# burritojustice/reporter

Measured on AMD Instinct MI355X. Metric: GPS points matched/sec (whole node) at 1/2/4/8 MI355X; % segment-ID agreement vs meili, higher is better.
Workload: dtype f32

## Files before the change

reporter_amd/csrc/engine.cpp:

```cpp
#include "engine.h"

#include "flush.h"

#include <algorithm>
#include <chrono>
#include <cmath>
#include <cstdlib>

#include <cstring>

namespace otm {

#define HIPCHK(x)                                                              \
  do {                                                                         \
    hipError_t e_ = (x);                                                       \
    if (e_ != hipSuccess) {                                                    \
      *err = std::string(#x) + ": " + hipGetErrorString(e_);                   \
      return OTM_EDEVICE;                                                      \
    }                                                                          \
  } while (0)

#define TRY(x)                    \
  do {                            \
    if (int rc_ = (x)) return rc_; \
// ... 87 lines not shown
  UP(OTMG_SHAPE_LON, s_lon);
  UP(OTMG_SHAPE_CUM, s_cum);
  UP(OTMG_SEG_ID, g_id);
  UP(OTMG_SEG_LEN, g_len);
  UP(OTMG_EDGE_HEAD_OUT, e_head_out);
  UP(OTMG_EDGE_HEAD_IN, e_head_in);
#undef UP
  {
    uint32_t tu[TURN_TABLE];
    for (int d = 0; d < TURN_TABLE; ++d) tu[d] = turn_units(E->mc.turn_penalty_factor, d);
    TRY(up(tu, sizeof tu, sizeof tu, E->dp.turn_units));
  }
  {
    const float* len = (const float*)E->host.section(OTMG_EDGE_LEN);
    std::vector<uint32_t> l64((size_t)h.n_edges + 1, 0u);
    for (int32_t e = 0; e < h.n_edges; ++e) l64[(size_t)e] = (uint32_t)std::floor((double)len[e] * 64.0 + 0.5);
    TRY(up(l64.data(), l64.size() * 4, l64.size() * 4, g.e_len64));
  }
  {
    const float* len = (const float*)E->host.section(OTMG_EDGE_LEN);
    const int32_t* seg = (const int32_t*)E->host.section(OTMG_EDGE_SEG);
    const int32_t* pos = (const int32_t*)E->host.section(OTMG_EDGE_SEG_POS);
    const uint8_t* fl = (const uint8_t*)E->host.section(OTMG_EDGE_FLAGS);
    const int64_t* way = (const int64_t*)E->host.section(OTMG_EDGE_WAY);
    std::vector<int64_t> ways(way, way + h.n_edges);
    std::sort(ways.begin(), ways.end());
    ways.erase(std::unique(ways.begin(), ways.end()), ways.end());
    if (ways.size() >= (size_t)INT32_MAX) {
      *err = "graph: more than 2^31 distinct way ids";
      return OTM_EINVAL;
    }
    std::vector<uint32_t> rec((size_t)h.n_edges * 4 + 4, 0u);
    for (int32_t e = 0; e < h.n_edges; ++e) {
      if (seg[e] >= 0 && (pos[e] < 0 || pos[e] >= (1 << 24))) {
        *err = "graph: an edge's position in its OSMLR segment exceeds 2^24";
        return OTM_EINVAL;
      }
      uint32_t* r = &rec[(size_t)e * 4];
      std::memcpy(&r[0], &len[e], 4);
      r[1] = (uint32_t)seg[e];
      r[2] = ((uint32_t)(seg[e] >= 0 ? pos[e] : 0) & 0xFFFFFFu) | ((uint32_t)fl[e] << 24);
      r[3] = (uint32_t)(std::lower_bound(ways.begin(), ways.end(), way[e]) - ways.begin());
    }
    if (ways.empty()) ways.push_back(0);
    TRY(up(rec.data(), rec.size() * 4, rec.size() * 4, g.e_rec));
    TRY(up(ways.data(), ways.size() * 8, ways.size() * 8, g.way_tab));
    const int32_t* from = (const int32_t*)E->host.section(OTMG_EDGE_FROM);
    std::vector<int32_t> fl2((size_t)h.n_edges * 2 + 2, 0);
    for (int32_t e = 0; e < h.n_edges; ++e) {
      fl2[(size_t)e * 2] = from[e];
      std::memcpy(&fl2[(size_t)e * 2 + 1], &len[e], 4);
    }
    TRY(up(fl2.data(), fl2.size() * 4, fl2.size() * 4, g.e_fl));
  }
  {
    const int m = E->grid_mult < 1 ? 1 : E->grid_mult;
    const int64_t* fo = (const int64_t*)E->host.section(OTMG_CELL_OFF);
    const uint32_t* fe = (const uint32_t*)E->host.section(OTMG_CELL_ENT);
    const int32_t R = (h.grid_rows + m - 1) / m, Cn = (h.grid_cols + m - 1) / m;
    std::vector<uint64_t> co_ent;
    const size_t nc = (size_t)R * (size_t)Cn + 1;
    std::vector<uint32_t> c32(nc, 0);
    std::vector<uint32_t> ent;
    if (m == 1) {
      if ((uint64_t)h.n_cell_entries >= (1ull << 32)) {
        *err = "graph: more than 2^32 cell entries (32-bit cell offsets)";
        return OTM_EINVAL;
      }
      for (size_t c = 0; c < nc; ++c) c32[c] = (uint32_t)fo[c];
      ent.assign(fe, fe + h.n_cell_entries);
    } else {
      co_ent.reserve((size_t)h.n_cell_entries);
      for (int32_t r = 0; r < h.grid_rows; ++r)
        for (int32_t c = 0; c < h.grid_cols; ++c) {
          const size_t f = (size_t)r * h.grid_cols + c;
          const uint64_t cc = (uint64_t)(r / m) * (uint64_t)Cn + (uint64_t)(c / m);
          for (int64_t q = fo[f]; q < fo[f + 1]; ++q) co_ent.push_back(cc << 32 | fe[q]);
        }
      std::sort(co_ent.begin(), co_ent.end());
      co_ent.erase(std::unique(co_ent.begin(), co_ent.end()), co_ent.end());
      if (co_ent.size() >= (1ull << 32)) {
        *err = "graph: more than 2^32 cell entries (32-bit cell offsets)";
        return OTM_EINVAL;
      }
      ent.resize(co_ent.size());
      for (size_t k = 0; k < co_ent.size(); ++k) {
        ent[k] = (uint32_t)co_ent[k];
        c32[(co_ent[k] >> 32) + 1]++;
      }
      for (size_t c = 0; c + 1 < nc; ++c) c32[c + 1] += c32[c];
      std::vector<uint64_t>().swap(co_ent);
    }
    E->grid_rows = R;
    E->grid_cols = Cn;
    E->grid_entries = (int64_t)ent.size();
    TRY(up(c32.data(), nc * 4, nc * 4, g.cell_off));
    TRY(up(ent.data(), ent.size() * 4, ent.size() * 4 + 16, g.cell_ent));
    const size_t ne = ent.size();
    const int32_t* soff = (const int32_t*)E->host.section(OTMG_EDGE_SHAPE_OFF);
    const float* slat = (const float*)E->host.section(OTMG_SHAPE_LAT);
    const float* slon = (const float*)E->host.section(OTMG_SHAPE_LON);
    std::vector<float> geo(ne * 4 + 4);
    for (size_t q = 0; q < ne; ++q) {
      const int32_t a = soff[ent[q] >> 4] + (int32_t)(ent[q] & 15u);
      geo[q * 4 + 0] = slat[a];
      geo[q * 4 + 1] = slon[a];
// ... 1766 lines not shown
```

reporter_amd/csrc/kernels.h:

```cpp
#pragma once
#include <hip/hip_runtime.h>

#include <cstddef>
#include <cstdint>

#include "otmatch.h"
#include "pairs.h"

namespace otm {

constexpr int KMAX = 32;
constexpr int KIN = 8;
static_assert(KIN == 4 || KIN == 8, "inline blocks of 4 or 8 slots (whole 16-B emission pieces)");
constexpr int KX = KMAX - KIN;
constexpr int MAX_HITS = 256;
constexpr int SEARCH_LIMIT = 98304;
constexpr int LDS_TABLE_CAP = 256;
constexpr int LDS_TABLE_LIMIT = 192;
constexpr int BIG_TABLE_LOG2 = 17;
constexpr int BIG_TABLE_CAP = 1 << BIG_TABLE_LOG2;
#ifndef OTM_BIG_SLOTS
#define OTM_BIG_SLOTS 512
#endif
constexpr int BIG_SLOTS = OTM_BIG_SLOTS;
constexpr int HUGE_SLOTS = 8;
constexpr int CAND_BIG_SLOTS = 64;
constexpr int HUGE_MAX_LOG2 = 27, CAND_MAX_LOG2 = 23;
__host__ __device__ inline int huge_limit(int log2) { return log2 > 2 ? 3 << (log2 - 2) : 0; }

struct DevGraph {
  const float *node_lat, *node_lon;
  const int32_t* out_off;
  const int32_t *e_from, *e_to;
  const float* e_len;
  const int32_t* e_shape_off;
  const int64_t* e_way;
  const int32_t *e_seg, *e_seg_pos;
  const uint8_t* e_flags;
  const float *s_lat, *s_lon, *s_cum;
  const uint64_t* g_id;
  const float* g_len;
  const uint32_t* cell_off;
  const uint32_t* cell_ent;
  const float4* ent_geo;
  const uint16_t *e_head_out, *e_head_in;
  const uint32_t* e_len64;
  const uint4* e_rec;
  const int2* e_fl;
  const int64_t* way_tab;
  int32_t n_nodes, n_edges, n_segments, grid_rows, grid_cols;
  double lat0, lon0, cell;
  float bb_lat0, bb_lon0, bb_inv_h, bb_inv_w;
};

#ifndef OTM_ORDER_BITS
#define OTM_ORDER_BITS 6
#endif
constexpr int ORDER_BITS = OTM_ORDER_BITS;
constexpr int ORDER_SIDE = 1 << ORDER_BITS;
constexpr int ORDER_TILES = ORDER_SIDE * ORDER_SIDE;
constexpr int ORDER_GROUPS = 8;
struct DevOrder {
  int32_t* item;
  int32_t* grp;
  uint16_t* tile;
  int32_t* tile_cnt;
  int32_t* cursor;
};

struct IdxRow {
  int64_t off;
  int32_t cnt;
  uint32_t cap;
};
#ifndef OTM_SRC_REC_BYTES
#define OTM_SRC_REC_BYTES 48
#endif
struct alignas(16) SrcRec {
  IdxRow edge;
  IdxRow node;
  int32_t from;
  int32_t len;
  int32_t pad[(OTM_SRC_REC_BYTES - 40) / 4];
};
static_assert(sizeof(SrcRec) == OTM_SRC_REC_BYTES && (OTM_SRC_REC_BYTES == 48 || OTM_SRC_REC_BYTES == 64),
              "source records of 48 or 64 bytes");
struct DevIndex {
  float rmax;
  uint32_t cmax;
  const IdxRow* row;
  const SrcRec* src;
  const uint4* slot;
  int load_pct;
};
constexpr int IDX_SLOT_BYTES = 16;
constexpr float INDEX_RMAX_CAP = 200000.0f;
constexpr uint32_t NODE_KEY = 0x80000000u;
constexpr uint32_t NONE_PRED = 0xFFFFFFFFu;
constexpr int NEAR_LEVELS = 3;
#ifndef OTM_INDEX_NEAR_FRACS
#define OTM_INDEX_NEAR_FRACS {0.45f}
// ... 298 lines not shown
```

reporter_amd/csrc/kernels.hip:

```cpp
#include <hip/hip_runtime.h>

#include <algorithm>
#include <cstdlib>
#include <type_traits>

#include <hipcub/hipcub.hpp>

#include "kernels.h"
#include "otmatch.h"

namespace otm {

namespace {

#define MPD_F 111319.4954833f
constexpr uint32_t EMPTY = 0xFFFFFFFFu;
constexpr unsigned long long LAB_NONE = ~0ull;
constexpr int TB = 64;
__device__ __forceinline__ void wave_sync() {
  __builtin_amdgcn_wave_barrier();
  asm volatile("" ::: "memory");
}

__device__ __forceinline__ float cos_deg(float deg) {
// ... 3 lines not shown
  c = c * x2 + 2.08767569878681e-09f;
  c = c * x2 - 2.755731922398589e-07f;
  c = c * x2 + 2.48015873015873e-05f;
  c = c * x2 - 0.001388888888888889f;
  c = c * x2 + 0.041666666666666664f;
  c = c * x2 - 0.5f;
  c = c * x2 + 1.0f;
  return c;
}

__device__ __forceinline__ float gc_dist(float la, float lo, float lb, float lob) {
  const float ls = MPD_F * cos_deg((la + lb) * 0.5f);
  const float dx = (lob - lo) * ls;
  const float dy = (lb - la) * MPD_F;
  return sqrtf(dx * dx + dy * dy);
}

__device__ __forceinline__ float seg_sqdist(float alat, float alon, float blat, float blon, float lat, float lon,
                                            float ls) {
  const float ax = (alon - lon) * ls;
  const float ay = (alat - lat) * MPD_F;
  const float bx = (blon - lon) * ls;
  const float by = (blat - lat) * MPD_F;
  const float vx = bx - ax;
  const float vy = by - ay;
  const float l2 = vx * vx + vy * vy;
  const float dot = ax * vx + ay * vy;
  float t = -dot / l2;
  t = t < 0.0f ? 0.0f : (t > 1.0f ? 1.0f : t);
  t = l2 > 0.0f ? t : 0.0f;
  const float px = ax + t * vx;
  const float py = ay + t * vy;
  return px * px + py * py;
}

typedef float float2_t __attribute__((ext_vector_type(2)));
__device__ __forceinline__ float seg_sqdist_pk(const float4 G, float2_t ll, float2_t sc) {
  const float2_t a = (float2_t{G.x, G.y} - ll) * sc;
  const float2_t b = (float2_t{G.z, G.w} - ll) * sc;
  const float2_t v = b - a;
  const float2_t vv = v * v;
  const float l2 = vv.y + vv.x;
  const float2_t av = a * v;
  const float dot = av.y + av.x;
  float t = -dot / l2;
  t = t < 0.0f ? 0.0f : (t > 1.0f ? 1.0f : t);
  t = l2 > 0.0f ? t : 0.0f;
  const float2_t p = a + t * v;
  const float2_t pp = p * p;
  return pp.y + pp.x;
}


struct ProjIn {
  float alon, alat, blon, blat, ca, cb, len;
  int32_t b, last;
};
__device__ __forceinline__ ProjIn proj_load(const DevGraph& g, int32_t e, int32_t k) {
  ProjIn in;
  const int32_t a = g.e_shape_off[e] + k, b = a + 1;
  in.last = g.e_shape_off[e + 1] - 1;
  in.alon = g.s_lon[a];
  in.alat = g.s_lat[a];
  in.blon = g.s_lon[b];
  in.blat = g.s_lat[b];
  in.ca = g.s_cum[a];
  in.cb = g.s_cum[b];
  in.len = g.e_len[e];
  in.b = b;
  return in;
}
__device__ __forceinline__ void proj_calc(const ProjIn& in, float lat, float lon, float ls, float& sqd,
                                          float& off_out, bool& at_end) {
  const float ax = (in.alon - lon) * ls;
  const float ay = (in.alat - lat) * MPD_F;
  const float bx = (in.blon - lon) * ls;
  const float by = (in.blat - lat) * MPD_F;
  const float vx = bx - ax;
  const float vy = by - ay;
  const float l2 = vx * vx + vy * vy;
  float t = 0.0f;
  if (l2 > 0.0f) {
    const float dot = ax * vx + ay * vy;
    t = -dot / l2;
    t = t < 0.0f ? 0.0f : (t > 1.0f ? 1.0f : t);
  }
  const float px = ax + t * vx;
  const float py = ay + t * vy;
  sqd = px * px + py * py;
  float off = in.ca + t * (in.cb - in.ca);
  off_out = off > in.len ? in.len : off;
  at_end = t == 1.0f && in.b == in.last;
}
__device__ __forceinline__ void project(const DevGraph& g, int32_t e, int32_t k, float lat, float lon, float ls,
                                        float& sqd, float& off_out, bool& at_end) {
  proj_calc(proj_load(g, e, k), lat, lon, ls, sqd, off_out, at_end);
}
__device__ __forceinline__ void project(const DevGraph& g, int32_t e, int32_t k, float lat, float lon, float ls,
                                        float& sqd, float& off_out) {
  bool at_end;
  project(g, e, k, lat, lon, ls, sqd, off_out, at_end);
}
__device__ __forceinline__ int32_t snap_node(const DevGraph& g, int32_t e, float off, bool at_end) {
  if (off == 0.0f) return g.e_from[e];
  if (at_end) {
    const int32_t v = g.e_to[e];
    if (g.out_off[v + 1] > g.out_off[v]) return v;
  }
  return -1;
}

__device__ __forceinline__ float probe_radius(const DevParams& P, float acc) {
  const float a = acc > 0.0f ? acc : P.gps_accuracy;
  const float r = a > P.search_radius ? a : P.search_radius;
  return r < P.max_search_radius ? r : P.max_search_radius;
}

__device__ __forceinline__ uint32_t fbits(float f) { return __float_as_uint(f); }
__device__ __forceinline__ float bitsf(uint32_t u) { return __uint_as_float(u); }
__device__ __forceinline__ uint32_t hash32(uint32_t x) { return x * 2654435761u; }

__device__ __forceinline__ void cadd(unsigned long long* c, unsigned long long v) {
  if (c && v) atomicAdd(c, v);
}

__device__ __forceinline__ int2 crec(const DevWork& w, int64_t p, int j) {
  return j < KIN ? w.cand_eo[p * KIN + j] : w.cand_xeo[p * KX + (j - KIN)];
}
__device__ __forceinline__ float cemis(const DevWork& w, int64_t p, int j) {
  return j < KIN ? w.cand_em[p * KIN + j] : w.cand_xem[p * KX + (j - KIN)];
}
__device__ __forceinline__ void cput(const DevWork& w, int64_t p, int j, int32_t e, float off, float em) {
  if (j < KIN) {
    w.cand_eo[p * KIN + j] = make_int2(e, __float_as_int(off));
    w.cand_em[p * KIN + j] = em;
  } else {
    w.cand_xeo[p * KX + (j - KIN)] = make_int2(e, __float_as_int(off));
    w.cand_xem[p * KX + (j - KIN)] = em;
  }
}

__device__ __forceinline__ uint32_t turn_deg(uint32_t hin, uint32_t hout) {
  int d = (int)hout - (int)hin;
  d += d < 0 ? 360 : 0;
  return (uint32_t)(d <= 180 ? d : 360 - d);
}
__device__ __forceinline__ float trans_cost(uint32_t units, float r, float gcv, float beta) {
  units = units > TURN_UNITS_MAX ? TURN_UNITS_MAX : units;
  const float tc = (float)units * 0.015625f;
  const float diff = fabsf(r - gcv);
  return (tc + diff) / beta;
}

constexpr uint32_t NO_HEAD = 0xFFFFu;
__device__ __forceinline__ bool cand_node(float off) { return off == 0.0f; }
__device__ __forceinline__ int32_t src_node(const DevGraph& g, int32_t e, float off) {
  return cand_node(off) ? g.e_from[e] : g.e_to[e];
}
__device__ __forceinline__ float src_start(const DevGraph& g, int32_t e, float off) {
  return cand_node(off) ? 0.0f : g.e_len[e] - off;
}
__device__ __forceinline__ uint32_t src_head(const DevGraph& g, int32_t e, float off) {
  return cand_node(off) ? NO_HEAD : (uint32_t)g.e_head_in[e];
}
// ... 375 lines not shown
      const uint32_t tot = e2 + (rg + 2 <= r1 ? qb[2] - qa[2] : 0u);
      const uint32_t b2 = qa[2] - e2, d1 = qa[1] - e1 - b2, d0 = qa[0] - (qa[1] - e1);
      if (CTR) ents += (unsigned long long)tot;
      auto entry_of = [&](uint32_t i) { return (size_t)(uint32_t)(i + b2 + (i < e2 ? d1 : 0u) + (i < e1 ? d0 : 0u)); };
      for (uint32_t done = 0, cn; done < tot && !spill; done += cn) {
        cn = tot - done < W ? tot - done : W;
        unsigned long long hit = 0ull;
        for (uint32_t k = 0; k < cn; k += CAND_INFL) {
          float4 G[CAND_INFL];
#pragma unroll
          for (int u = 0; u < CAND_INFL; ++u) G[u] = g.ent_geo[entry_of(done + k + (u == 0 || k + u < cn ? u : 0))];
          __builtin_amdgcn_sched_barrier(0);
          uint32_t bits = 0u;
#pragma unroll
          for (int u = 0; u < CAND_INFL; ++u) {
            const float sq = seg_sqdist_pk(G[u], pll, psc);
            bits |= ((uint32_t)(u == 0 || k + u < cn) & (uint32_t)(sq <= r2)) << u;
          }
          hit |= (unsigned long long)bits << k;
        }
        while (hit != 0ull && !spill) {
          const size_t qx = entry_of(done + (uint32_t)(__ffsll(hit) - 1));
          hit &= hit - 1ull;
          const bool two = hit != 0ull;
          const size_t qy = two ? entry_of(done + (uint32_t)(__ffsll(hit) - 1)) : qx;
          hit &= hit - 1ull;
          const uint32_t ent0 = g.cell_ent[qx], ent1 = g.cell_ent[qy];
          const float4 G0 = g.ent_geo[qx], G1 = g.ent_geo[qy];
          __builtin_amdgcn_sched_barrier(0);
          const float s0 = seg_sqdist_pk(G0, pll, psc), s1 = seg_sqdist_pk(G1, pll, psc);
          insert(ent0, s0);
          if (two && !spill) insert(ent1, s1);
        }
      }
    }
    if (spill) {
      spill_push<CTR_CAND_WAVE>(w, (int32_t)p);
      continue;
    }
    float offr[CAND_LANE_CAP];
    uint32_t perm = 076543210u;
#pragma unroll
    for (int m0 = 0; m0 < CAND_LANE_CAP; m0 += SNAP_B) {
#pragma unroll
      for (int u = 0; u < SNAP_B; ++u) offr[m0 + u] = 0.0f;
      if (m0 >= n) continue;
      uint32_t em[SNAP_B];
      ProjIn pin[SNAP_B];
#pragma unroll
      for (int u = 0; u < SNAP_B; ++u) {
        em[u] = m0 + u < n ? E[(m0 + u) * S] : 0u;
        if (m0 + u < n) pin[u] = proj_load(g, (int32_t)(em[u] >> 4), (int32_t)(em[u] & 15u));
      }
      int32_t vx[SNAP_B];
      bool node0[SNAP_B], at_end[SNAP_B];
      float offv[SNAP_B];
#pragma unroll
      for (int u = 0; u < SNAP_B; ++u) {
        vx[u] = 0;
        node0[u] = at_end[u] = false;
        offv[u] = 0.0f;
        if (m0 + u < n) {
          float sqd, off;
          proj_calc(pin[u], lat, lon, ls, sqd, off, at_end[u]);
          offv[u] = off;
          node0[u] = off == 0.0f;
          const int32_t e = (int32_t)(em[u] >> 4);
          if (node0[u] || at_end[u]) vx[u] = node0[u] ? g.e_from[e] : g.e_to[e];
        }
      }
#pragma unroll
      for (int u = 0; u < SNAP_B; ++u) {
        if (node0[u] || at_end[u]) {
          const int32_t o0 = g.out_off[vx[u]], o1 = g.out_off[vx[u] + 1];
          if (node0[u] || o1 > o0) {
            E[(m0 + u) * S] = NODE_ENT | ((uint32_t)o0 << 4);
            offv[u] = 0.0f;
          }
        }
        offr[m0 + u] = offv[u];
      }
    }
    for (int m = 0; m < n; ++m) {
      const uint32_t key = E[m * S];
      if (!(key & NODE_ENT)) continue;
      int f = -1;
      for (int t = 0; t < m; ++t)
        if (E[t * S] == key) f = t;
      if (f >= 0) {
        const float qm = Q[m * S];
        if (qm < Q[f * S]) Q[f * S] = qm;
        --n;
        E[m * S] = E[n * S];
        Q[m * S] = Q[n * S];
        perm = (perm & ~(7u << (3 * m))) | ((perm >> (3 * n)) & 7u) << (3 * m);
        --m;
      }
    }
    const int K = n < P.max_candidates ? n : P.max_candidates;
    const float ds = (2.0f * P.sigma_z) * P.sigma_z;
    for (int j = 0; j < K; ++j) {
      int m = j;
      float qm = Q[j * S];
      uint32_t em = E[j * S];
      for (int t = j + 1; t < n; ++t) {
        const float qt = Q[t * S];
        const uint32_t et = E[t * S];
        const uint32_t xt = (et & ~NODE_ENT) >> 4, xm = (em & ~NODE_ENT) >> 4;
        if (qt < qm || (qt == qm && (xt < xm || (xt == xm && et > em)))) {
          m = t;
          qm = qt;
          em = et;
        }
      }
      if (m != j) {
        Q[m * S] = Q[j * S];
        E[m * S] = E[j * S];
        Q[j * S] = qm;
        E[j * S] = em;
        const uint32_t x = ((perm >> (3 * m)) ^ (perm >> (3 * j))) & 7u;
        perm ^= x << (3 * m) | x << (3 * j);
      }
    }
    int4* eo4 = (int4*)(w.cand_eo + p * KIN);
    float4* em4 = (float4*)(w.cand_em + p * KIN);
    float emv[4];
#pragma unroll
    for (int j = 0; j < (CAND_LANE_CAP > KIN ? CAND_LANE_CAP : KIN); j += 2) {
      if (j >= KIN && j >= K) break;
      int32_t e2[2];
      float o2[2];
#pragma unroll
      for (int u = 0; u < 2; ++u) {
// ... 103 lines not shown
    const float r = probe_radius(P, pr.z);
    const float r2 = r * r;
    const float ls = MPD_F * cos_deg(lat);
    const float dlat = r / MPD_F;
    const float dlon = r / ls;
    const double la_lo = ((double)lat - (double)dlat - g.lat0) / g.cell;
    const double la_hi = ((double)lat + (double)dlat - g.lat0) / g.cell;
    const double lo_lo = ((double)lon - (double)dlon - g.lon0) / g.cell;
    const double lo_hi = ((double)lon + (double)dlon - g.lon0) / g.cell;
    const double R = g.grid_rows, Cn = g.grid_cols;
    int r0 = 0, r1 = -1, c0 = 0, c1 = -1;
    if (!(la_hi < 0.0 || lo_hi < 0.0 || la_lo >= R || lo_lo >= Cn)) {
      r0 = la_lo < 0.0 ? 0 : (int)floor(la_lo);
      r1 = la_hi >= R ? (int)R - 1 : (int)floor(la_hi);
      c0 = lo_lo < 0.0 ? 0 : (int)floor(lo_lo);
      c1 = lo_hi >= Cn ? (int)Cn - 1 : (int)floor(lo_hi);
    }
    const int ncols = c1 - c0 + 1;
    const int ncells = (r1 - r0 + 1) * ncols;
    for (int i = lane; i < hcap; i += TB) {
      Mem<BIG>::st(&hkey[i], (uint32_t)EMPTY);
      Mem<BIG>::st(&hval[i], (unsigned long long)LAB_NONE);
    }
    if (lane == 0) {
      s_count = 0;
      s_over = 0;
      s_n = 0;
    }
    __syncthreads();
    unsigned long long scanned = 0;
    for (int cb = 0; cb < ncells; cb += TB) {
      const int c = cb + lane;
      int cnt = 0;
      int64_t cs = 0;
      if (c < ncells) {
        const int rr = r0 + c / ncols, cc = c0 + c % ncols;
        const size_t cidx = (size_t)rr * (size_t)g.grid_cols + (size_t)cc;
        cs = g.cell_off[cidx];
        cnt = (int)(g.cell_off[cidx + 1] - cs);
      }
      const int incl = wave_incl_scan(cnt, lane);
      const int total = __shfl(incl, 63, 64);
      cexcl[lane] = incl - cnt;
      cstart[lane] = cs;
      __syncthreads();
      const int nc_here = min(TB, ncells - cb);
      for (int gi = lane; gi < total; gi += TB) {
        int lo = 0, hi = nc_here - 1;
        while (lo < hi) {
          const int mid = (lo + hi + 1) >> 1;
          if (cexcl[mid] <= gi) lo = mid;
          else hi = mid - 1;
        }
        const uint32_t ent = g.cell_ent[cstart[lo] + (gi - cexcl[lo])];
        const int32_t e = (int32_t)(ent >> 4), k = (int32_t)(ent & 15u);
        float sqd, off;
        project(g, e, k, lat, lon, ls, sqd, off);
        if (!(sqd <= r2)) continue;
        uint32_t slot = hash32((uint32_t)e) >> (32 - hlog2);
        bool placed = false;
        for (int probe = 0; probe < hcap; ++probe) {
          const uint32_t old = atomicCAS(&hkey[slot], EMPTY, (uint32_t)e);
          if (old == EMPTY) {
            if (atomicAdd(&s_count, 1) >= max_hits) s_over = 1;
            placed = true;
            break;
          }
          if (old == (uint32_t)e) {
            placed = true;
            break;
          }
          slot = (slot + 1) & (uint32_t)(hcap - 1);
        }
        if (!placed) {
          s_over = 1;
          continue;
        }
        atomicMin(&hval[slot], ((unsigned long long)fbits(sqd) << 32) | (unsigned long long)k);
      }
      scanned += (unsigned long long)total;
      __syncthreads();
    }
    if (s_over) {
      if (lane == 0) {
        if (!BIG) {
          spill_push<CTR_CAND_BIG>(w, (int32_t)p);
        } else if (w.cand_final) {
          w.ncand[p] = 0;
          atomicCAS(&w.trace_err[w.pt_trace[p]], 0, OTM_TERR_CAND_OVERFLOW);
        } else {
          w.ncand[p] = 0;
          w.counters_i32[CTR_GROW_CAND] = 1;
          *w.abort = 1;
        }
      }
      __syncthreads();
      continue;
    }
    for (int i = lane; i < hcap; i += TB) {
      const uint32_t hk = Mem<BIG>::ld(&hkey[i]);
      if (hk != EMPTY) {
        const unsigned long long hv = Mem<BIG>::ld(&hval[i]);
        const int idx = atomicAdd(&s_n, 1);
        Mem<BIG>::st(&skey[idx],
                     (hv & 0xFFFFFFFF00000000ull) | ((unsigned long long)hk << 5) | ((hv & 15ull) << 1));
      }
    }
    __syncthreads();
    for (int i = lane; i < hcap; i += TB) {
      Mem<BIG>::st(&hkey[i], (uint32_t)EMPTY);
      Mem<BIG>::st(&hval[i], (unsigned long long)LAB_NONE);
    }
    if (lane == 0) s_count = 0;
    __syncthreads();
    const int n0 = s_n;
    for (int idx = lane; idx < n0; idx += TB) {
      const unsigned long long key = Mem<BIG>::ld(&skey[idx]);
      const int32_t e = (int32_t)(((uint32_t)key) >> 5);
      float sqd, off;
      bool at_end;
      project(g, e, (int32_t)((key >> 1) & 15ull), lat, lon, ls, sqd, off, at_end);
      const int32_t v = snap_node(g, e, off, at_end);
      if (v < 0) {
        Mem<BIG>::st(&skey[idx], key | 1ull);
        atomicAdd(&s_count, 1);
      } else {
        Mem<BIG>::st(&skey[idx], (unsigned long long)LAB_NONE);
        const uint32_t rep = (uint32_t)g.out_off[v];
        uint32_t slot = hash32(rep) >> (32 - hlog2);
        while (true) {
          const uint32_t old = atomicCAS(&hkey[slot], EMPTY, rep);
          if (old == EMPTY || old == rep) break;
          slot = (slot + 1) & (uint32_t)(hcap - 1);
        }
        atomicMin(&hval[slot], (key & 0xFFFFFFFF00000000ull) | (unsigned long long)idx);
      }
    }
    __syncthreads();
    for (int i = lane; i < hcap; i += TB) {
      const uint32_t hk = Mem<BIG>::ld(&hkey[i]);
      if (hk != EMPTY) {
        const unsigned long long hv = Mem<BIG>::ld(&hval[i]);
        Mem<BIG>::st(&skey[(int)(hv & 0xFFFFFFFFull)], (hv & 0xFFFFFFFF00000000ull) | ((unsigned long long)hk << 5));
        atomicAdd(&s_count, 1);
      }
    }
    __syncthreads();
    const int ns = n0;
    const int n = s_count;
    int N = 1;
    while (N < ns) N <<= 1;
    for (int i = ns + lane; i < N; i += TB) Mem<BIG>::st(&skey[i], (unsigned long long)LAB_NONE);
    __syncthreads();
    for (int kk = 2; kk <= N; kk <<= 1) {
      for (int j = kk >> 1; j > 0; j >>= 1) {
        for (int i = lane; i < N; i += TB) {
          const int ixj = i ^ j;
          if (ixj > i) {
            const unsigned long long x = Mem<BIG>::ld(&skey[i]), y = Mem<BIG>::ld(&skey[ixj]);
            const bool up = (i & kk) == 0;
            if ((x > y) == up) {
              Mem<BIG>::st(&skey[i], y);
              Mem<BIG>::st(&skey[ixj], x);
            }
          }
        }
        __syncthreads();
      }
    }
    const int K = n < P.max_candidates ? n : P.max_candidates;
    if (lane < K) {
      const unsigned long long key = Mem<BIG>::ld(&skey[lane]);
      const int32_t e = (int32_t)(((uint32_t)key) >> 5);
      float sqd = bitsf((uint32_t)(key >> 32)), off = 0.0f;
      if (key & 1ull) project(g, e, (int32_t)((key >> 1) & 15ull), lat, lon, ls, sqd, off);
      const float ds = (2.0f * P.sigma_z) * P.sigma_z;
      cput(w, p, lane, e, off, sqd / ds);
    } else if (lane < KIN) {
      cput(w, p, lane, -1, 0.0f, INFINITY);
    }
    if (lane == 0) {
// ... 2878 lines not shown
    otm_trace_result r;
    r.error_kind = w.trace_err[t];
    r.seg_off = (int32_t)o.seg_base[t];
    r.seg_cnt = o.seg_cnt[t];
    r.rep_off = r.seg_off;
    const otm_segment* G = o.segments + r.seg_off;
    otm_report_rec* REP = o.reports + r.rep_off;
    const bool fits = r.seg_cnt <= REPW_CAP;
    if (fits && r.error_kind == 0) {
      const unsigned long long* gw = (const unsigned long long*)G;
      for (int k = lane; k < r.seg_cnt * SW; k += TB) sSeg[k] = gw[k];
    }
    __syncthreads();
    if (lane == 0) {
      const int nrep = report_walk(t, b, rc, w, fits ? (const otm_segment*)sSeg : G, r, REP);
      r.rep_cnt = nrep;
      sN = nrep;
      if (w.ctr && r.code == 200) {
        cadd(&w.ctr->segments_out, (unsigned long long)r.seg_cnt);
        cadd(&w.ctr->reports_out, (unsigned long long)nrep);
      }
      o.traces[t] = r;
      o.rep_cnt[t] = nrep;
      __threadfence_block();
    }
    __syncthreads();
    const int nrep = sN;
    for (int k = lane; k < nrep; k += TB) report_pass(o, r.seg_off, r.seg_cnt, REP[k]);
    __syncthreads();
  }
}

struct RoutePiece {
  int32_t edge;
  float o0, o1, xs;
};
__device__ float interp_pos(const DevGraph& g, const DevBatch& b, const DevParams& P, const DevWork& w, int64_t q,
                            int64_t p, int64_t k) {
  const int2 ci = w.chosen[q], cj = w.chosen[p];
  const int32_t ei = ci.x, ej = cj.x;
  const float oi = __int_as_float(ci.y), oj = __int_as_float(cj.y);
  const int32_t poff = w.path_off[p], plen = w.path_len[p];
  const bool has0 = !cand_node(oi);
  const int npc = (has0 ? 1 : 0) + plen + (cand_node(oj) ? 0 : 1);
  const float start = src_start(g, ei, oi);
  const float ds = (2.0f * P.sigma_z) * P.sigma_z;
  const float lat = b.lat[k], lon = b.lon[k];
  const float ls = MPD_F * cos_deg(lat);
  const float gcd = gc_dist(b.lat[q], b.lon[q], lat, lon);
  float best = INFINITY, bpos = -1.0f, dd = 0.0f;
  for (int m = 0; m < npc; ++m) {
    RoutePiece pc;
    const int pk = m - (has0 ? 1 : 0);
    if (has0 && m == 0) {
      pc = RoutePiece{ei, oi, g.e_len[ei], 0.0f};
    } else if (pk < plen) {
      const int32_t e = w.path_pool[poff + pk];
      const float len = g.e_len[e];
      pc = RoutePiece{e, 0.0f, len, start + dd};
      dd = dd + len;
    } else {
      pc = RoutePiece{ej, 0.0f, oj, start + dd};
    }
    const int32_t s0 = g.e_shape_off[pc.edge], nsh = g.e_shape_off[pc.edge + 1] - s0 - 1;
    float bsq = INFINITY, boff = 0.0f;
    for (int sg = 0; sg < nsh; ++sg) {
      float sqd, off;
      project(g, pc.edge, sg, lat, lon, ls, sqd, off);
      if (sqd < bsq) {
        bsq = sqd;
        boff = off;
      }
    }
    if (!(boff >= pc.o0 && boff <= pc.o1)) continue;
    const float pos = pc.xs + (boff - pc.o0);
    const float cost = bsq / ds + fabsf(pos - gcd) / P.beta;
    if (cost < best) {
      best = cost;
      bpos = pos;
    }
  }
  return bpos;
}

__global__ __launch_bounds__(256) void k_seg_bound(DevGraph g, DevBatch b, DevParams P, DevWork w, int64_t* tb) {
  const int64_t k = (int64_t)blockIdx.x * blockDim.x + threadIdx.x;
  if (k == b.n_points) fold_snap(w, SNAP_AFTER_ROUTE, false);
  if (*w.abort) return;
  const int lane = threadIdx.x & 63;
  int64_t v = 0;
  int32_t t = -1;
  if (k < b.n_points) {
    t = w.pt_trace[k];
    if (w.is_col[k]) {
      if (w.state[k] >= 0) {
        const int32_t pl = w.path_len[k];
        v = 2 + (pl > 0 ? pl : 0);
      }
    } else {
      const int32_t q = w.prevc[k];
      const int32_t p = q >= 0 ? w.nextc[q] : -1;
      if (p >= 0 && w.col_prev[p] == q && !w.chain_start[p] && w.state[p] >= 0 && w.path_len[p] >= 0 &&
          w.trace_err[t] == 0) {
        const int2 ci = w.chosen[q], cj = w.chosen[p];
        if (!same_edge_step(ci.x, __int_as_float(ci.y), cj.x, __int_as_float(cj.y)))
          w.ipos[k] = interp_pos(g, b, P, w, q, p, k);
      }
    }
  }
#pragma unroll
  for (int d = 1; d < 64; d <<= 1) {
    const int64_t vn = __shfl_down(v, d, 64);
    const int32_t tn = __shfl_down(t, d, 64);
    if (lane + d < 64 && tn == t) v += vn;
  }
  const int32_t tp = __shfl_up(t, 1, 64);
  if (t >= 0 && (lane == 0 || tp != t) && v != 0) atomicAdd((unsigned long long*)&tb[t], (unsigned long long)v);
}

__global__ __launch_bounds__(TB) void k_compact(int32_t n_traces, DevOut o, const int32_t* seg_off, const int32_t* way_off,
                                                const int32_t* rep_off, otm_segment* so, int64_t* wo,
                                                otm_report_rec* ro, otm_trace_result* to) {
  const int lane = threadIdx.x;
  const otm_trace_result* TR = o.traces;
  const otm_segment* SI = o.segments;
  const otm_report_rec* RI = o.reports;
// ... 37 lines not shown
    if (lane == 63) {
      ws[0][wv] = i0;
      ws[1][wv] = i1;
      ws[2][wv] = i2;
    }
    __syncthreads();
    int b0 = 0, b1 = 0, b2 = 0, z0 = 0, z1 = 0, z2 = 0;
    for (int k = 0; k < 16; ++k) {
      const int w0 = ws[0][k], w1 = ws[1][k], w2 = ws[2][k];
      if (k < wv) {
        b0 += w0;
        b1 += w1;
        b2 += w2;
      }
      z0 += w0;
      z1 += w1;
      z2 += w2;
    }
    if (i < n) {
      o0[i] = carry0 + b0 + i0 - s0;
      o1[i] = carry1 + b1 + i1 - s1;
      o2[i] = carry2 + b2 + i2 - s2;
    }
    carry0 += z0;
    carry1 += z1;
    carry2 += z2;
    __syncthreads();
  }
  if (t == 0) {
    o0[n] = carry0;
    o1[n] = carry1;
    o2[n] = carry2;
  }
}

__device__ int2 interp_foot(const DevGraph& g, const DevBatch& b, const DevParams& P, const DevWork& w, int64_t q,
                            int64_t p, int64_t k) {
  const int2 ci = w.chosen[q], cj = w.chosen[p];
  const int32_t ei = ci.x, ej = cj.x;
  const float oi = __int_as_float(ci.y), oj = __int_as_float(cj.y);
  const int32_t poff = w.path_off[p], plen = w.path_len[p];
  const bool has0 = !cand_node(oi);
  const int npc = (has0 ? 1 : 0) + plen + (cand_node(oj) ? 0 : 1);
  const float start = src_start(g, ei, oi);
  const float ds = (2.0f * P.sigma_z) * P.sigma_z;
  const float lat = b.lat[k], lon = b.lon[k];
  const float ls = MPD_F * cos_deg(lat);
  const float gcd = gc_dist(b.lat[q], b.lon[q], lat, lon);
  float best = INFINITY, dd = 0.0f, bo = 0.0f;
  int32_t be = -1;
  for (int m = 0; m < npc; ++m) {
    RoutePiece pc;
    const int pk = m - (has0 ? 1 : 0);
    if (has0 && m == 0) {
      pc = RoutePiece{ei, oi, g.e_len[ei], 0.0f};
    } else if (pk < plen) {
      const int32_t e = w.path_pool[poff + pk];
      const float len = g.e_len[e];
      pc = RoutePiece{e, 0.0f, len, start + dd};
      dd = dd + len;
    } else {
      pc = RoutePiece{ej, 0.0f, oj, start + dd};
    }
    const int32_t s0 = g.e_shape_off[pc.edge], nsh = g.e_shape_off[pc.edge + 1] - s0 - 1;
    float bsq = INFINITY, boff = 0.0f;
    for (int sg = 0; sg < nsh; ++sg) {
      float sqd, off;
      project(g, pc.edge, sg, lat, lon, ls, sqd, off);
      if (sqd < bsq) {
        bsq = sqd;
        boff = off;
      }
    }
    if (!(boff >= pc.o0 && boff <= pc.o1)) continue;
    const float pos = pc.xs + (boff - pc.o0);
    const float cost = bsq / ds + fabsf(pos - gcd) / P.beta;
    if (cost < best) {
      best = cost;
      be = pc.edge;
      bo = boff;
    }
  }
  return make_int2(be, __float_as_int(bo));
}

__device__ float edge_foot(const DevGraph& g, const DevBatch& b, int32_t e, int64_t k, float lo, float hi) {
  const float lat = b.lat[k], lon = b.lon[k];
  const float ls = MPD_F * cos_deg(lat);
  const int32_t nsh = g.e_shape_off[e + 1] - g.e_shape_off[e] - 1;
  float bsq = INFINITY, boff = 0.0f;
  for (int sg = 0; sg < nsh; ++sg) {
    float sqd, off;
    project(g, e, sg, lat, lon, ls, sqd, off);
    if (sqd < bsq) {
      bsq = sqd;
      boff = off;
    }
  }
  return boff < lo ? lo : (boff > hi ? hi : boff);
}

__global__ __launch_bounds__(TB) void k_points(DevGraph g, DevBatch b, DevParams P, DevWork w,
                                               otm_matched_point* out) {
  if (*w.abort) return;
  const int lane = threadIdx.x;
  for (int32_t t = blockIdx.x; t < b.n_traces; t += gridDim.x) {
    const int64_t a = b.trace_off[t];
    const int n = (int)(b.trace_off[t + 1] - a);
    const bool ok = w.trace_err[t] == 0;
    float carry = -1.0f;
    for (int c0 = 0; c0 < n; c0 += TB) {
      const int pl = c0 + lane;
      const bool in = pl < n;
      const int64_t k = a + pl;
      bool col = false;
      uint32_t flags = 0;
      int32_t edge = -1;
      float off = 0.0f, x = -1.0f;
      if (in) {
        col = w.is_col[k] != 0;
        if (col) {
          flags = OTM_PT_COLUMN;
          if (ok && w.state[k] >= 0) {
            const int2 c = w.chosen[k];
            edge = c.x;
            off = __int_as_float(c.y);
            flags |= OTM_PT_MATCHED | (cand_node(off) ? OTM_PT_NODE : 0u) | (w.chain_start[k] ? OTM_PT_CHAIN_START : 0u);
          }
        } else if (ok) {
          const int32_t q = w.prevc[k];
          const int32_t p = q >= 0 ? w.nextc[q] : -1;
          if (p >= 0 && w.col_prev[p] == q && !w.chain_start[p] && w.state[p] >= 0 && w.path_len[p] >= 0) {
            const int2 ci = w.chosen[q], cj = w.chosen[p];
            const float oi = __int_as_float(ci.y), oj = __int_as_float(cj.y);
            if (same_edge_step(ci.x, oi, cj.x, oj)) {
              edge = ci.x;
              off = edge_foot(g, b, edge, k, oi < oj ? oi : oj, oi < oj ? oj : oi);
              flags = OTM_PT_MATCHED | OTM_PT_SAME_EDGE;
            } else {
              x = w.ipos[k];
              if (x >= 0.0f) {
                const int2 f = interp_foot(g, b, P, w, q, p, k);
                edge = f.x;
                off = __int_as_float(f.y);
                flags = OTM_PT_MATCHED | OTM_PT_ROUTE;
              } else {
                x = -1.0f;
              }
            }
          }
        }
// ... 319 lines not shown
    "k_columns",       "spatial_order",  "k_cand_lane",    "k_candidates",     "k_links",         "scan_trans_off",  "k_trans_sub",
    "k_trans_wide",    "k_transitions",  "k_transitions_big", "k_viterbi",      "k_route_index",
    "k_route",         "k_route_big",    "k_seg_bound",      "scan_seg_bound",  "k_segments",       "k_report"};

namespace {
constexpr int SPILL_GRID = 4096;
#ifndef OTM_WIDE_GRID
#define OTM_WIDE_GRID 8192
#endif
constexpr int WIDE_GRID = OTM_WIDE_GRID;
}

#define TIMED(k, launch) \
  do {                   \
    mk.begin(k, s);      \
    launch;              \
    mk.end(k, s);        \
  } while (0)

void launch_columns(const DevGraph& g, const DevBatch& b, const DevParams& p, DevWork& w, hipStream_t s,
                    const Marks& mk) {
  if (w.ord.tile_cnt) (void)hipMemsetAsync(w.ord.tile_cnt, 0, ORDER_TILES * 4, s);
  TIMED(KN_COLUMNS, hipLaunchKernelGGL(k_columns, dim3(grid_for(b.n_traces, 1, WAVE_GRID_CAP)), dim3(TB), 0, s, g,
                                       b, p, w));
}
static int order_grid(int64_t n, int per_block, int cap) {
  const int64_t per_group = (n + ORDER_GROUPS - 1) / ORDER_GROUPS;
  int64_t gb = (per_group + per_group / 4 + per_block - 1) / per_block;
  if (gb < 1) gb = 1;
  int64_t gtot = gb * ORDER_GROUPS;
  if (gtot > cap) gtot = cap / ORDER_GROUPS * ORDER_GROUPS;
  return (int)gtot;
}

void launch_order(const DevBatch& b, DevWork& w, hipStream_t s, const Marks& mk) {
  mk.begin(KN_ORDER, s);
  hipLaunchKernelGGL(k_order_plan, dim3(1), dim3(1024), 0, s, w.ord.tile_cnt, w.ord.cursor, w.ord.grp);
  hipLaunchKernelGGL(k_order_scatter, dim3(grid_for(b.n_points, 256, 8192)), dim3(256), 0, s, b, w, w.ord.tile,
                     w.ord.cursor, w.ord.item);
  mk.end(KN_ORDER, s);
}

void launch_candidates(const DevGraph& g, const DevBatch& b, const DevParams& p, DevWork& w, hipStream_t s,
                       const Marks& mk, int from) {
  if (from < RESUME_CAND_BIG) {
    if (w.ctr)
      TIMED(KN_CAND_LANE, hipLaunchKernelGGL(k_cand_lane<true>, dim3(order_grid(b.n_points, CAND_TB, 1 << 30)),
                                             dim3(CAND_TB), 0, s, g, b, p, w));
    else
      TIMED(KN_CAND_LANE, hipLaunchKernelGGL(k_cand_lane<false>, dim3(order_grid(b.n_points, CAND_TB, 1 << 30)),
                                             dim3(CAND_TB), 0, s, g, b, p, w));
  }
  mk.begin(KN_CAND_WAVE, s);
  if (from < RESUME_CAND_BIG) hipLaunchKernelGGL(k_candidates<false>, dim3(4096), dim3(TB), 0, s, g, b, p, w);
  hipLaunchKernelGGL(k_candidates<true>, dim3(CAND_BIG_SLOTS), dim3(TB), 0, s, g, b, p, w);
  mk.end(KN_CAND_WAVE, s);
}
void launch_links(const DevBatch& b, const DevParams& p, DevWork& w, hipStream_t s, const Marks& mk) {
  TIMED(KN_LINKS, hipLaunchKernelGGL(k_links, dim3(grid_for(b.n_points + 1, 256, 1 << 30)), dim3(256), 0, s, b, p,
                                     w));
}
__global__ __launch_bounds__(256) void k_expand_compact(const int64_t* trace_off, const int64_t* tbase,
                                                        const int32_t* dt, const int16_t* acc16, double* time,
                                                        float* acc, int32_t n_traces) {
  const int wv = threadIdx.x >> 6, lane = threadIdx.x & 63;
  for (int64_t t = (int64_t)blockIdx.x * 4 + wv; t < n_traces; t += (int64_t)gridDim.x * 4) {
    const int64_t a = trace_off[t], e = trace_off[t + 1], base = tbase[t];
    for (int64_t i = a + lane; i < e; i += 64) {
      time[i] = (double)(base + (int64_t)dt[i]);
      acc[i] = (float)acc16[i];
    }
  }
}
void launch_expand_compact(const int64_t* trace_off, const int64_t* tbase, const int32_t* dt, const int16_t* acc16,
                           double* time, float* acc, int32_t n_traces, hipStream_t s) {
  if (n_traces <= 0) return;
  hipLaunchKernelGGL(k_expand_compact, dim3(grid_for(((int64_t)n_traces + 3) / 4, 1, 1 << 20)), dim3(256), 0, s,
                     trace_off, tbase, dt, acc16, time, acc, n_traces);
}
void launch_status(const int32_t* abort, const int64_t* ttotal, const int32_t* counters, BatchStatus* out,
                   hipStream_t s) {
  hipLaunchKernelGGL(k_status, dim3(1), dim3(64), 0, s, abort, ttotal, counters, out);
}
void launch_transitions(const DevGraph& g, const DevBatch& b, const DevParams& p, DevWork& w, hipStream_t s,
                        const Marks& mk, int sub, int from) {
  if (from >= RESUME_TRANS_HUGE) {
    mk.begin(KN_TRANS_GLOBAL, s);
    hipLaunchKernelGGL(k_transitions<2>, dim3(HUGE_SLOTS), dim3(TB), 0, s, g, b, p, w);
    mk.end(KN_TRANS_GLOBAL, s);
    return;
  }
  const int per = TB / sub;
  const int grid = order_grid((b.n_points + per - 1) / per, 1, TRANS_GRID_CAP);
  if (sub == 8) {
    TIMED(KN_TRANS_INDEX, hipLaunchKernelGGL((k_trans_sub<8, false>), dim3(grid), dim3(TB), 0, s, g, b, p, w));
    TIMED(KN_TRANS_WIDE, hipLaunchKernelGGL((k_trans_sub<16, true>), dim3(WIDE_GRID), dim3(TB), 0, s, g, b, p, w));
  } else {
    TIMED(KN_TRANS_INDEX, hipLaunchKernelGGL((k_trans_sub<16, false>), dim3(grid), dim3(TB), 0, s, g, b, p, w));
    mk.begin(KN_TRANS_WIDE, s);
    mk.end(KN_TRANS_WIDE, s);
  }
  TIMED(KN_TRANS_WAVE, hipLaunchKernelGGL(k_transitions<0>, dim3(SPILL_GRID), dim3(TB), 0, s, g, b, p, w));
  mk.begin(KN_TRANS_GLOBAL, s);
  hipLaunchKernelGGL(k_transitions<1>, dim3(BIG_SLOTS), dim3(TB), 0, s, g, b, p, w);
  hipLaunchKernelGGL(k_transitions<2>, dim3(HUGE_SLOTS), dim3(TB), 0, s, g, b, p, w);
  mk.end(KN_TRANS_GLOBAL, s);
}
// ... 148 lines not shown
```

Before: 1.670 billion.

## Pack shape points and per-edge projection records into interleaved float4/int4 arrays

```diff
diff --git a/reporter_amd/csrc/engine.cpp b/reporter_amd/csrc/engine.cpp
--- a/reporter_amd/csrc/engine.cpp
+++ b/reporter_amd/csrc/engine.cpp
@@ -163,6 +163,30 @@
       std::memcpy(&fl2[(size_t)e * 2 + 1], &len[e], 4);
     }
     TRY(up(fl2.data(), fl2.size() * 4, fl2.size() * 4, g.e_fl));
+    const int32_t* to = (const int32_t*)E->host.section(OTMG_EDGE_TO);
+    const int32_t* soff = (const int32_t*)E->host.section(OTMG_EDGE_SHAPE_OFF);
+    const int32_t* ooff = (const int32_t*)E->host.section(OTMG_NODE_OUT_OFF);
+    const float* slat = (const float*)E->host.section(OTMG_SHAPE_LAT);
+    const float* slon = (const float*)E->host.section(OTMG_SHAPE_LON);
+    const float* scum = (const float*)E->host.section(OTMG_SHAPE_CUM);
+    const size_t ns = h.sec[OTMG_SHAPE_LAT].bytes / 4;
+    std::vector<int32_t> pt(ns * 4 + 4, -1), pr((size_t)h.n_edges * 4 + 4, 0);
+    for (size_t a = 0; a < ns; ++a) {
+      std::memcpy(&pt[a * 4 + 0], &slat[a], 4);
+      std::memcpy(&pt[a * 4 + 1], &slon[a], 4);
+      std::memcpy(&pt[a * 4 + 2], &scum[a], 4);
+    }
+    for (int32_t e = 0; e < h.n_edges; ++e) {
+      const int32_t last = soff[e + 1] - 1;
+      pt[(size_t)last * 4 + 3] = ooff[to[e] + 1] > ooff[to[e]] ? ooff[to[e]] : -2;
+      int32_t* r = &pr[(size_t)e * 4];
+      r[0] = soff[e];
+      r[1] = last;
+      std::memcpy(&r[2], &len[e], 4);
+      r[3] = ooff[from[e]];
+    }
+    TRY(up(pt.data(), pt.size() * 4, pt.size() * 4, g.s_pt));
+    TRY(up(pr.data(), pr.size() * 4, pr.size() * 4, g.e_proj));
   }
   {
     const int m = E->grid_mult < 1 ? 1 : E->grid_mult;
diff --git a/reporter_amd/csrc/kernels.h b/reporter_amd/csrc/kernels.h
--- a/reporter_amd/csrc/kernels.h
+++ b/reporter_amd/csrc/kernels.h
@@ -47,6 +47,8 @@
   const uint32_t* e_len64;
   const uint4* e_rec;
   const int2* e_fl;
+  const int4* e_proj;
+  const float4* s_pt;
   const int64_t* way_tab;
   int32_t n_nodes, n_edges, n_segments, grid_rows, grid_cols;
   double lat0, lon0, cell;
diff --git a/reporter_amd/csrc/kernels.hip b/reporter_amd/csrc/kernels.hip
--- a/reporter_amd/csrc/kernels.hip
+++ b/reporter_amd/csrc/kernels.hip
@@ -79,23 +79,30 @@
 }
 
 
+constexpr int32_t PT_INNER = -1;
 struct ProjIn {
   float alon, alat, blon, blat, ca, cb, len;
-  int32_t b, last;
+  int32_t rep_from, end;
 };
+__device__ __forceinline__ ProjIn proj_points(const DevGraph& g, const int4 er, int32_t k) {
+  ProjIn in;
+  const int32_t a = er.x + k;
+  typedef float float3_t __attribute__((ext_vector_type(3)));
+  const float3_t pa = *(const float3_t*)(g.s_pt + a);
+  const float4 pb = g.s_pt[a + 1];
+  in.alat = pa.x;
+  in.alon = pa.y;
+  in.ca = pa.z;
+  in.blat = pb.x;
+  in.blon = pb.y;
+  in.cb = pb.z;
+  in.end = __float_as_int(pb.w);
+  in.len = __int_as_float(er.z);
+  in.rep_from = er.w;
+  return in;
+}
 __device__ __forceinline__ ProjIn proj_load(const DevGraph& g, int32_t e, int32_t k) {
-  ProjIn in;
-  const int32_t a = g.e_shape_off[e] + k, b = a + 1;
-  in.last = g.e_shape_off[e + 1] - 1;
-  in.alon = g.s_lon[a];
-  in.alat = g.s_lat[a];
-  in.blon = g.s_lon[b];
-  in.blat = g.s_lat[b];
-  in.ca = g.s_cum[a];
-  in.cb = g.s_cum[b];
-  in.len = g.e_len[e];
-  in.b = b;
-  return in;
+  return proj_points(g, g.e_proj[e], k);
 }
 __device__ __forceinline__ void proj_calc(const ProjIn& in, float lat, float lon, float ls, float& sqd,
                                           float& off_out, bool& at_end) {
@@ -117,7 +124,25 @@
   sqd = px * px + py * py;
   float off = in.ca + t * (in.cb - in.ca);
   off_out = off > in.len ? in.len : off;
-  at_end = t == 1.0f && in.b == in.last;
+  at_end = t == 1.0f && in.end != PT_INNER;
+}
+__device__ __forceinline__ int32_t snap_rep(const ProjIn& in, float off, bool at_end) {
+  return off == 0.0f ? in.rep_from : (at_end ? in.end : -1);
+}
+__device__ __forceinline__ void project_edge(const DevGraph& g, const int4 er, float lat, float lon, float ls,
+                                             float& bsq, float& boff) {
+  bsq = INFINITY;
+  boff = 0.0f;
+  const int32_t nsh = er.y - er.x;
+  for (int sg = 0; sg < nsh; ++sg) {
+    float sqd, off;
+    bool at_end;
+    proj_calc(proj_points(g, er, sg), lat, lon, ls, sqd, off, at_end);
+    if (sqd < bsq) {
+      bsq = sqd;
+      boff = off;
+    }
+  }
 }
 __device__ __forceinline__ void project(const DevGraph& g, int32_t e, int32_t k, float lat, float lon, float ls,
                                         float& sqd, float& off_out, bool& at_end) {
@@ -128,15 +153,6 @@
   bool at_end;
   project(g, e, k, lat, lon, ls, sqd, off_out, at_end);
 }
-__device__ __forceinline__ int32_t snap_node(const DevGraph& g, int32_t e, float off, bool at_end) {
-  if (off == 0.0f) return g.e_from[e];
-  if (at_end) {
-    const int32_t v = g.e_to[e];
-    if (g.out_off[v + 1] > g.out_off[v]) return v;
-  }
-  return -1;
-}
-
 __device__ __forceinline__ float probe_radius(const DevParams& P, float acc) {
   const float a = acc > 0.0f ? acc : P.gps_accuracy;
   const float r = a > P.search_radius ? a : P.search_radius;
@@ -618,33 +634,19 @@
         em[u] = m0 + u < n ? E[(m0 + u) * S] : 0u;
         if (m0 + u < n) pin[u] = proj_load(g, (int32_t)(em[u] >> 4), (int32_t)(em[u] & 15u));
       }
-      int32_t vx[SNAP_B];
-      bool node0[SNAP_B], at_end[SNAP_B];
-      float offv[SNAP_B];
 #pragma unroll
       for (int u = 0; u < SNAP_B; ++u) {
-        vx[u] = 0;
-        node0[u] = at_end[u] = false;
-        offv[u] = 0.0f;
         if (m0 + u < n) {
           float sqd, off;
-          proj_calc(pin[u], lat, lon, ls, sqd, off, at_end[u]);
-          offv[u] = off;
-          node0[u] = off == 0.0f;
-          const int32_t e = (int32_t)(em[u] >> 4);
-          if (node0[u] || at_end[u]) vx[u] = node0[u] ? g.e_from[e] : g.e_to[e];
-        }
-      }
-#pragma unroll
-      for (int u = 0; u < SNAP_B; ++u) {
-        if (node0[u] || at_end[u]) {
-          const int32_t o0 = g.out_off[vx[u]], o1 = g.out_off[vx[u] + 1];
-          if (node0[u] || o1 > o0) {
-            E[(m0 + u) * S] = NODE_ENT | ((uint32_t)o0 << 4);
-            offv[u] = 0.0f;
+          bool at_end;
+          proj_calc(pin[u], lat, lon, ls, sqd, off, at_end);
+          const int32_t rep = snap_rep(pin[u], off, at_end);
+          if (rep >= 0) {
+            E[(m0 + u) * S] = NODE_ENT | ((uint32_t)rep << 4);
+            off = 0.0f;
           }
-        }
-        offr[m0 + u] = offv[u];
+          offr[m0 + u] = off;
+        }
       }
     }
     for (int m = 0; m < n; ++m) {
@@ -854,10 +856,11 @@
           if (cexcl[mid] <= gi) lo = mid;
           else hi = mid - 1;
         }
-        const uint32_t ent = g.cell_ent[cstart[lo] + (gi - cexcl[lo])];
+        const int64_t q = cstart[lo] + (gi - cexcl[lo]);
+        const uint32_t ent = g.cell_ent[q];
+        const float4 G = g.ent_geo[q];
         const int32_t e = (int32_t)(ent >> 4), k = (int32_t)(ent & 15u);
-        float sqd, off;
-        project(g, e, k, lat, lon, ls, sqd, off);
+        const float sqd = seg_sqdist(G.x, G.y, G.z, G.w, lat, lon, ls);
         if (!(sqd <= r2)) continue;
         uint32_t slot = hash32((uint32_t)e) >> (32 - hlog2);
         bool placed = false;
@@ -921,14 +924,15 @@
       const int32_t e = (int32_t)(((uint32_t)key) >> 5);
       float sqd, off;
       bool at_end;
-      project(g, e, (int32_t)((key >> 1) & 15ull), lat, lon, ls, sqd, off, at_end);
-      const int32_t v = snap_node(g, e, off, at_end);
+      const ProjIn pin = proj_load(g, e, (int32_t)((key >> 1) & 15ull));
+      proj_calc(pin, lat, lon, ls, sqd, off, at_end);
+      const int32_t v = snap_rep(pin, off, at_end);
       if (v < 0) {
         Mem<BIG>::st(&skey[idx], key | 1ull);
         atomicAdd(&s_count, 1);
       } else {
         Mem<BIG>::st(&skey[idx], (unsigned long long)LAB_NONE);
-        const uint32_t rep = (uint32_t)g.out_off[v];
+        const uint32_t rep = (uint32_t)v;
         uint32_t slot = hash32(rep) >> (32 - hlog2);
         while (true) {
           const uint32_t old = atomicCAS(&hkey[slot], EMPTY, rep);
@@ -3913,26 +3917,20 @@
   for (int m = 0; m < npc; ++m) {
     RoutePiece pc;
     const int pk = m - (has0 ? 1 : 0);
+    const bool mid = !(has0 && m == 0) && pk < plen;
+    const int32_t e = has0 && m == 0 ? ei : (mid ? w.path_pool[poff + pk] : ej);
+    const int4 er = g.e_proj[e];
+    const float len = __int_as_float(er.z);
     if (has0 && m == 0) {
-      pc = RoutePiece{ei, oi, g.e_len[ei], 0.0f};
-    } else if (pk < plen) {
-      const int32_t e = w.path_pool[poff + pk];
-      const float len = g.e_len[e];
+      pc = RoutePiece{e, oi, len, 0.0f};
+    } else if (mid) {
       pc = RoutePiece{e, 0.0f, len, start + dd};
       dd = dd + len;
     } else {
-      pc = RoutePiece{ej, 0.0f, oj, start + dd};
-    }
-    const int32_t s0 = g.e_shape_off[pc.edge], nsh = g.e_shape_off[pc.edge + 1] - s0 - 1;
-    float bsq = INFINITY, boff = 0.0f;
-    for (int sg = 0; sg < nsh; ++sg) {
-      float sqd, off;
-      project(g, pc.edge, sg, lat, lon, ls, sqd, off);
-      if (sqd < bsq) {
-        bsq = sqd;
-        boff = off;
-      }
-    }
+      pc = RoutePiece{e, 0.0f, oj, start + dd};
+    }
+    float bsq, boff;
+    project_edge(g, er, lat, lon, ls, bsq, boff);
     if (!(boff >= pc.o0 && boff <= pc.o1)) continue;
     const float pos = pc.xs + (boff - pc.o0);
     const float cost = bsq / ds + fabsf(pos - gcd) / P.beta;
@@ -4076,26 +4074,20 @@
   for (int m = 0; m < npc; ++m) {
     RoutePiece pc;
     const int pk = m - (has0 ? 1 : 0);
+    const bool mid = !(has0 && m == 0) && pk < plen;
+    const int32_t e = has0 && m == 0 ? ei : (mid ? w.path_pool[poff + pk] : ej);
+    const int4 er = g.e_proj[e];
+    const float len = __int_as_float(er.z);
     if (has0 && m == 0) {
-      pc = RoutePiece{ei, oi, g.e_len[ei], 0.0f};
-    } else if (pk < plen) {
-      const int32_t e = w.path_pool[poff + pk];
-      const float len = g.e_len[e];
+      pc = RoutePiece{e, oi, len, 0.0f};
+    } else if (mid) {
       pc = RoutePiece{e, 0.0f, len, start + dd};
       dd = dd + len;
     } else {
-      pc = RoutePiece{ej, 0.0f, oj, start + dd};
-    }
-    const int32_t s0 = g.e_shape_off[pc.edge], nsh = g.e_shape_off[pc.edge + 1] - s0 - 1;
-    float bsq = INFINITY, boff = 0.0f;
-    for (int sg = 0; sg < nsh; ++sg) {
-      float sqd, off;
-      project(g, pc.edge, sg, lat, lon, ls, sqd, off);
-      if (sqd < bsq) {
-        bsq = sqd;
-        boff = off;
-      }
-    }
+      pc = RoutePiece{e, 0.0f, oj, start + dd};
+    }
+    float bsq, boff;
+    project_edge(g, er, lat, lon, ls, bsq, boff);
     if (!(boff >= pc.o0 && boff <= pc.o1)) continue;
     const float pos = pc.xs + (boff - pc.o0);
     const float cost = bsq / ds + fabsf(pos - gcd) / P.beta;
@@ -4111,16 +4103,8 @@
 __device__ float edge_foot(const DevGraph& g, const DevBatch& b, int32_t e, int64_t k, float lo, float hi) {
   const float lat = b.lat[k], lon = b.lon[k];
   const float ls = MPD_F * cos_deg(lat);
-  const int32_t nsh = g.e_shape_off[e + 1] - g.e_shape_off[e] - 1;
-  float bsq = INFINITY, boff = 0.0f;
-  for (int sg = 0; sg < nsh; ++sg) {
-    float sqd, off;
-    project(g, e, sg, lat, lon, ls, sqd, off);
-    if (sqd < bsq) {
-      bsq = sqd;
-      boff = off;
-    }
-  }
+  float bsq, boff;
+  project_edge(g, g.e_proj[e], lat, lon, ls, bsq, boff);
   return boff < lo ? lo : (boff > hi ? hi : boff);
 }
 
@@ -4546,7 +4530,11 @@
                                              dim3(CAND_TB), 0, s, g, b, p, w));
   }
   mk.begin(KN_CAND_WAVE, s);
-  if (from < RESUME_CAND_BIG) hipLaunchKernelGGL(k_candidates<false>, dim3(4096), dim3(TB), 0, s, g, b, p, w);
+#ifndef OTM_CAND_WAVE_GRID
+#define OTM_CAND_WAVE_GRID 4096
+#endif
+  if (from < RESUME_CAND_BIG)
+    hipLaunchKernelGGL(k_candidates<false>, dim3(OTM_CAND_WAVE_GRID), dim3(TB), 0, s, g, b, p, w);
   hipLaunchKernelGGL(k_candidates<true>, dim3(CAND_BIG_SLOTS), dim3(TB), 0, s, g, b, p, w);
   mk.end(KN_CAND_WAVE, s);
 }
```

After: 1.703 billion, median of 6. 2.0% higher.
